# qcNPU/LifeLong-CLIP

Measured on AMD Instinct MI355X. Metric: images/sec/GPU (ViT-B/16 fwd+bwd, bs=256) + online A_AUC on CIFAR-100, higher is better.
Workload: dtype bf16

## Files before the change

include/lc_clip.h:

```cpp
#ifndef LC_CLIP_H
#define LC_CLIP_H
#include <hip/hip_runtime_api.h>
#include <stdint.h>

#ifdef __cplusplus
extern "C" {
#endif

#define LC_OK 0
#define LC_EINVAL (-1)
#define LC_ELAUNCH (-2)
#define LC_EUNSUPPORTED (-3)

#define LC_EPI_BF16 0
#define LC_EPI_F32 1
#define LC_EPI_RESID 2
#define LC_EPI_GELU 3
#define LC_EPI_GELU_BWD 4
#define LC_EPI_BF16_F32 5
#define LC_EPI_GELU_D 6
#define LC_EPI_MUL 7
#define LC_EPI_GELU_D_Q8 12
#define LC_EPI_MUL_Q8 13
#define LC_EPI_RESID16 14
// ... 214 lines not shown
                               const float* beta, void* y, long ldy, float* mean, float* rstd,
                               long row_mul, long row_add);

int lc_adapter_bwd(hipStream_t stream, int M, int D, const void* gout, long ldg, const void* h,
                   const void* WuT, const void* WdT, float scale, float keep, void* dpre,
                   void* dz, long ldz);

int lc_adapter_bwd_set_form(int fused);

int lc_adapter_wgrad(hipStream_t stream, int M, int D, const void* gout, long ldg, const void* h,
                     const void* z, long ldz, const void* dpre, float scale, float* dWu,
                     float* dbu, float* dWd, float* dbd);
int lc_adapter_wgrad_ws(hipStream_t stream, int M, int D, const void* gout, long ldg,
                        const void* h, const void* z, long ldz, const void* dpre, float scale,
                        float* dWu, float* dbu, float* dWd, float* dbd, void* ws, long ws_bytes);

int lc_check_finite(hipStream_t stream, long n, const float* g, int* flag);

int lc_adamw(hipStream_t stream, long n, float* p, const float* g, float* m, float* v, float lr,
             float b1, float b2, float eps, float wd, int step, const int* skip,
             const long long* step_dev);

int lc_counter_add(hipStream_t stream, int n, long long* ctr, long long delta);

int lc_adam_step_advance(hipStream_t stream, long long* ctr, const int* skip);

int lc_l2norm_rows(hipStream_t stream, int R, int E, const float* f, long ldf, float* out,
                   float* norms);

int lc_clip_head(hipStream_t stream, int B, int C, int E, const float* img_n, const float* txt_n,
// ... 66 lines not shown
int lc_adapter_ln_fwd_f16(hipStream_t stream, int M, int D, const void* z, long ldz, const void* Wd,
                          const float* bd, const void* Wu, const float* bu, float scale, float keep,
                          unsigned long long seed, const unsigned long long* seed_dev,
                          const float* resid, float* xout, long ldx, void* hout,
                          const float* gamma, const float* beta, void* y, long ldy, float* mean,
                          float* rstd);
int lc_adapter_bwd_f16(hipStream_t stream, int M, int D, const void* gout, long ldg, const void* h,
                       const void* WuT, const void* WdT, float scale, float keep, void* dpre,
                       void* dz, long ldz);
int lc_adapter_wgrad_f16(hipStream_t stream, int M, int D, const void* gout, long ldg, const void* h,
                         const void* z, long ldz, const void* dpre, float scale, float* dWu,
                         float* dbu, float* dWd, float* dbd);
int lc_adapter_wgrad_ws_f16(hipStream_t stream, int M, int D, const void* gout, long ldg,
                            const void* h, const void* z, long ldz, const void* dpre, float scale,
                            float* dWu, float* dbu, float* dWd, float* dbd, void* ws, long ws_bytes);
int lc_patchify_f16(hipStream_t stream, int n_img, int res, int patch, const float* img, void* out);
int lc_vit_embed_ln_f16(hipStream_t stream, int n_img, int n_patch, int D, const float* patch,
                        const float* cls, const float* pos, const float* ln_pre_w,
                        const float* ln_pre_b, float* x0, const float* ln1_w, const float* ln1_b,
                        void* y, float* mean1, float* rstd1);


int lc_mvp_select(hipStream_t stream, int B, int P, int W, int K, const float* query, long ldq,
                  const float* key, long ldk, const float* count, int64_t* idx, float* dist,
                  float* qnorm, float* knorm, unsigned long long* hist);

int lc_mvp_simloss(hipStream_t stream, int B, int P, int W, int K, int contrastiv,
                   const float* key, long ldk, const float* count, const int64_t* idx,
                   const float* dist, const float* knorm, float* kcos, float* rawgd, float* rawW,
                   float* coef, float* loss);
// ... 44 lines not shown
```

lifelong-clip_amd/csrc/gemm.hip:

```cpp
#include "lc_common.h"
#include <stdlib.h>
#include <type_traits>

enum {
  EPI_BF16 = 0,
  EPI_F32 = 1,
  EPI_RESID = 2,
  EPI_GELU = 3,
  EPI_GELU_BWD = 4,
  EPI_BF16_F32 = 5,
  EPI_GELU_D = 6,
  EPI_MUL = 7,
  EPI_AD_DOWN = 8,
  EPI_AD_UP = 9,
  EPI_AD_MASK = 10,
  EPI_AD_ADD = 11,
  EPI_GELU_D_Q8 = 12,
  EPI_MUL_Q8 = 13,
  EPI_RESID16 = 14,
};

namespace {

constexpr int BK = 64;


LC_DEV int swz(int row, int chunk) { return chunk ^ ((row >> 1) & 7); }

LC_DEV void tile_coords(int tile, int tiles_m, int tiles_n, int gm, int& tm, int& tn) {
  if (gm <= 1) {
    tm = tile / tiles_n;
    tn = tile % tiles_n;
    return;
  }
// ... 249 lines not shown
      } else if constexpr (EPI == EPI_AD_ADD) {
#pragma unroll
        for (int i = 0; i < CPL; ++i) w[i] = bfv(xb, i) + v[i];
        store_bf(rs0, ldo0, m, w);
      }
    }
  }
}

template <int BM, int BN, int WM, int WN, int STAGES, int EPI>
__global__ void __launch_bounds__(64 * WM * WN, (WM * WN == 4 ? 2 : 1))
gemm_nt_kernel(int M, int N, int K, const bf16_t* __restrict__ A, long lda,
               const bf16_t* __restrict__ B, long ldb, const float* __restrict__ bias,
               float alpha, void* __restrict__ out0, long ldo0, void* __restrict__ out1,
               long ldo1, const void* __restrict__ aux, long ldaux, EpiParams ep) {
  constexpr int NW = WM * WN;
  constexpr int TM = BM / WM / 16;
  constexpr int TN = BN / WN / 16;
  constexpr int STAGE_BYTES = (BM + BN) * 128;
  constexpr int LOADS = (BM + BN) / 8 / NW;
  constexpr int PASS_MAX = STAGES == 1 ? 16 : 32;
  constexpr int EPI_BYTES = NW * ((BM / WM) % PASS_MAX == 0 ? PASS_MAX : 16) * (BN / WN + 4) * 4;
  constexpr int SMEM = STAGES * STAGE_BYTES > EPI_BYTES ? STAGES * STAGE_BYTES : EPI_BYTES;
  __shared__ __attribute__((aligned(16))) char smem[SMEM];

  const int tid = threadIdx.x, lane = tid & 63, wave = tid >> 6;
  const int wm = wave / WN, wn = wave % WN;

  const int tiles_n = N / BN;
  const int tiles_m = (M + BM - 1) / BM;
// ... 72 lines not shown

    int cur = 0;
    for (int kt = 0; kt < nk; ++kt) {
      const int pre = kt + STAGES - 1;
      int pbuf = cur + STAGES - 1;
      if (pbuf >= STAGES) pbuf -= STAGES;
      if (pre < nk) stage(pbuf, pre);
      compute(smem + cur * STAGE_BYTES);
      if (pre < nk) wait_vmcnt<LOADS * (STAGES - 2)>();
      else wait_vmcnt<0>();
      __builtin_amdgcn_s_barrier();
      cur = cur + 1 == STAGES ? 0 : cur + 1;
    }
  }

  store_tile<BM, BN, WM, WN, EPI, PASS_MAX>(acc, smem, SMEM, m0, n0, M, bias, alpha, out0, ldo0,
                                            out1, ldo1, aux, ldaux, ep);
}

LC_DEV int swz64(int row, int chunk) { return chunk ^ (((row >> 3) & 1) << 1); }

struct SplitK {
  int dp_tiles;
  int splits;
  float* slabs;
  int* tickets;
};

LC_DEV void splitk_slice(int s_id, int tail_tiles, int S, int& tail, int& split) {
#ifdef LC_SPLITK_SPREAD
  tail = s_id / S;
  split = s_id % S;
// ... 871 lines not shown
        if (n1 < N1 && n2 < N2) atomicAdd(C + (long)n1 * ldc + n2, acc[i][j][r] * alpha);
      }
}

struct TnProb {
  const bf16_t* W;
  long ldw;
  const bf16_t* S;
  long lds;
  float* C;
  long ldc;
  int Nw, ns, trans;
  float alpha;
  float* cs_w;
  float cs_w_scale;
  float* cs_s;
  float cs_s_scale;
  int M, n_chunks, n_tiles, wgs;
  float* part;
  int pw;
  const float* div;
  int w16;
};
LC_DEV float tn_unscale(const TnProb& p, float v) { return p.div ? v / *p.div : v; }

template <int PW>
struct TnGeom {
  static constexpr int ROWB = PW * 2;
  static constexpr int WB = 64 * ROWB;
  static constexpr int SLOT = WB + 64 * 128;
#ifndef TNW256_STAGES
#define TNW256_STAGES 3
#endif
  static constexpr int STAGES = PW == 256 ? TNW256_STAGES : 5;
  static constexpr int WPW = WB / 1024 / 8;
  static constexpr int LOADS = WPW + 1;
  static constexpr int TI = PW / 64;
};

__host__ __device__ inline int tn_pslot(int pw) { return pw * 64 + pw + 64; }

template <int PW>
__global__ void __launch_bounds__(512, 1)
gemm_tn_wide_kernel(TnProb p0, TnProb p1) {
  using Geo = TnGeom<PW>;
  constexpr int STAGES = Geo::STAGES, SLOT = Geo::SLOT, LOADS = Geo::LOADS, TI = Geo::TI;
  constexpr int ROWB = Geo::ROWB, LPRW = ROWB / 16, RPP = 64 / LPRW;
  constexpr int PSLOT = PW * 64 + PW + 64;
  __shared__ __attribute__((aligned(16))) char smem[STAGES * SLOT];
  const bool second = (int)blockIdx.x >= p0.wgs;
  const TnProb& p = second ? p1 : p0;
  const int bid = second ? blockIdx.x - p0.wgs : blockIdx.x;
  const int tid = threadIdx.x, lane = tid & 63;
  const int wave = __builtin_amdgcn_readfirstlane(tid >> 6);
  const int wn = wave & 3, wsv = wave >> 2;
  const int g = lane >> 4, t = lane & 15;
  const int tile = bid % p.n_tiles, cidx = bid / p.n_tiles;
  const int nblk = (p.M + 63) / 64;
  float* slot = p.part ? p.part + (long)(tile * p.n_chunks + cidx) * PSLOT : nullptr;
  if (cidx >= nblk) {
    if (slot)
      for (int e = tid; e < PSLOT; e += 512) slot[e] = 0.f;
    return;
  }
  const int nsteps = (nblk - 1 - cidx) / p.n_chunks + 1;
  auto blk_row = [&](int s) { return (cidx + s * p.n_chunks) * 64; };
  const int nw_pad = (p.Nw + 63) & ~63;
  const bool do_csw = p.cs_w != nullptr && wsv == 0;
  const bool do_css = p.cs_s != nullptr && tile == 0 && wn == 0;

  auto dma = [&](int s) {
    char* sl = smem + (s % STAGES) * SLOT;
    const int r0 = blk_row(s);
#pragma unroll
    for (int i = 0; i < Geo::WPW; ++i) {
      const int piece = wave * Geo::WPW + i;
      const int lr = piece * RPP + lane / LPRW;
      const int pc = lane % LPRW;
      const int c = (((pc >> 1) ^ swz_w(lr)) << 1) | (pc & 1);
      const int r = min(r0 + lr, p.M - 1);
      int col = tile * PW + c * 8;
      col = col < nw_pad ? col : col - 64;
      glds16(p.W + (long)r * p.ldw + col, sl + piece * 1024);
    }
    {
      const int piece = wave;
      const int lr = piece * 8 + (lane >> 3);
      const int pc = lane & 7;
      const int c = (((pc >> 1) ^ swz_s(lr)) << 1) | (pc & 1);
      const int r = min(r0 + lr, p.M - 1);
      glds16(p.S + (long)r * p.lds + c * 8, sl + Geo::WB + piece * 1024);
    }
  };

  f32x4 acc[TI][2], csw[TI], css[2];
#pragma unroll
  for (int i = 0; i < TI; ++i) {
    csw[i] = f32x4{0.f, 0.f, 0.f, 0.f};
#pragma unroll
    for (int j = 0; j < 2; ++j) acc[i][j] = f32x4{0.f, 0.f, 0.f, 0.f};
  }
  css[0] = css[1] = f32x4{0.f, 0.f, 0.f, 0.f};
  const short one = LC_ONE16;

#pragma unroll
  for (int s = 0; s < STAGES - 1; ++s)
    if (s < nsteps) dma(s);
  for (int s = 0; s < nsteps; ++s) {
    const int ahead = min(nsteps - 1 - s, STAGES - 2);
    if (STAGES > 4 && ahead >= 3) wait_vmcnt<3 * LOADS>();
    else if (STAGES > 3 && ahead == 2) wait_vmcnt<2 * LOADS>();
    else if (ahead >= 1) wait_vmcnt<LOADS>();
    else wait_vmcnt<0>();
    lds_barrier();
    if (s + STAGES - 1 < nsteps) dma(s + STAGES - 1);
    const uint32_t sw = lds_addr(smem + (s % STAGES) * SLOT);
    const uint32_t ss = sw + Geo::WB;
    const int valid = p.M - blk_row(s);
    bf16x8 fwk[2][TI], fsk[2][2];
#pragma unroll
    for (int ks = 0; ks < 2; ++ks) {
      const int row = ks * 32 + g * 8 + (t >> 2);
#pragma unroll
      for (int i = 0; i < TI; ++i)
        fwk[ks][i] = tr_frag_asm<ROWB>(sw, row, wn * (PW / 4) + i * 16 + (t & 3) * 4);
#pragma unroll
      for (int j = 0; j < 2; ++j)
        fsk[ks][j] = tr_frag_asm<128>(ss, row, wsv * 32 + j * 16 + (t & 3) * 4);
    }
    lds_wait0();
    if (p.w16) {
// ... 148 lines not shown
    LC_NT_CASE(EPI_RESID)
    LC_NT_CASE(EPI_RESID16)
    LC_NT_CASE(EPI_GELU)
    LC_NT_CASE(EPI_GELU_BWD)
    LC_NT_CASE(EPI_BF16_F32)
    LC_NT_CASE(EPI_GELU_D)
    LC_NT_CASE(EPI_MUL)
    LC_NT_CASE(EPI_AD_DOWN)
    LC_NT_CASE(EPI_AD_UP)
    LC_NT_CASE(EPI_AD_MASK)
    LC_NT_CASE(EPI_AD_ADD)
    default:
      return LC_EINVAL;
  }
#undef LC_NT_CASE
  LC_LAUNCH_RET();
}

int g_split_mode = -1;

int cu_count() {
  static int cus[64] = {0};
  int dev = 0;
  if (hipGetDevice(&dev) != hipSuccess || dev < 0 || dev >= 64) return 256;
  if (cus[dev] == 0) {
    int n = 0;
    if (hipDeviceGetAttribute(&n, hipDeviceAttributeMultiprocessorCount, dev) != hipSuccess || n <= 0)
      n = 256;
    cus[dev] = n;
  }
// ... 392 lines not shown
  LC_CHECK_ARG(bias == nullptr || ((uintptr_t)bias & 15) == 0);
  if ((epi != EPI_BF16 && epi != EPI_F32) || alpha != 1.0f) return LC_EUNSUPPORTED;
  const FullRoute r = full_route(epi, bias, alpha, M_full, N, K, ws, ws_bytes);
  if (!r.ok) return LC_EUNSUPPORTED;
  const int S = r.sk.splits, nt = K / 64;
  const int tiles = ((M_full + 255) / 256) * (N / 256);
  float* part = nullptr;
  if (S > 1) {
    if (LC_SPLITK_TICKET_BYTES + (long)S * n * N * 4 > ws_bytes) return LC_EUNSUPPORTED;
    part = reinterpret_cast<float*>(static_cast<char*>(ws) + LC_SPLITK_TICKET_BYTES);
  }
  const EpiParams ep{nullptr, 0, 1.0f, 1.0f, 0, g_dbg};
  int rc = lc_gemm_nt_ex(stream, epi, n, N, K, A, lda, B, ldb, bias, alpha, out, ldo, nullptr, 0,
                         nullptr, 0, ep, nullptr, 0);
  if (rc != LC_OK || S == 1) return rc;
  for (int s = 0; s < S; ++s) {
    const int tb = s * nt / S, te = (s + 1) * nt / S;
    rc = lc_gemm_nt_ex(stream, EPI_F32, n, N, (te - tb) * 64,
                       static_cast<const bf16_t*>(A) + (long)tb * 64, lda,
                       static_cast<const bf16_t*>(B) + (long)tb * 64, ldb, nullptr, 1.0f,
                       part + (long)s * n * N, N, nullptr, 0, nullptr, 0, ep, nullptr, 0);
    if (rc != LC_OK) return rc;
  }
  dim3 grid(tiles - r.sk.dp_tiles), block(256);
  if (epi == EPI_BF16)
    hipLaunchKernelGGL((gemm_rows_fixup_kernel<EPI_BF16>), grid, block, 0, stream, n, N, M_full,
                       mul, add, r.group_m, r.sk.dp_tiles, S, part, bias, alpha, out, ldo);
  else
    hipLaunchKernelGGL((gemm_rows_fixup_kernel<EPI_F32>), grid, block, 0, stream, n, N, M_full,
                       mul, add, r.group_m, r.sk.dp_tiles, S, part, bias, alpha, out, ldo);
  LC_LAUNCH_RET();
}

int lc_gemm_nt(hipStream_t stream, int epi, int M, int N, int K, const void* A, long lda,
               const void* B, long ldb, const float* bias, float alpha, void* out0, long ldo0,
               void* out1, long ldo1, const void* aux, long ldaux) {
  return lc_gemm_nt_ws(stream, epi, M, N, K, A, lda, B, ldb, bias, alpha, out0, ldo0, out1, ldo1,
                       aux, ldaux, nullptr, 0);
// ... 116 lines not shown
                     static_cast<const bf16_t*>(A), lda, static_cast<const bf16_t*>(B), ldb, alpha,
                     C, ldc, colsum, colsum_scale);
  LC_LAUNCH_RET();
}

int lc_adapter_wgrad(hipStream_t stream, int M, int D, const void* gout, long ldg, const void* h,
                     const void* z, long ldz, const void* dpre, float scale, float* dWu,
                     float* dbu, float* dWd, float* dbd) {
  return lc_adapter_wgrad_ws(stream, M, D, gout, ldg, h, z, ldz, dpre, scale, dWu, dbu, dWd, dbd,
                             nullptr, 0);
}

static int adapter_wgrad(hipStream_t stream, int M, int D, const void* gout, long ldg,
                         const void* h, const void* z, long ldz, const void* dpre, float scale,
                         float* dWu, float* dbu, float* dWd, float* dbd, void* ws, long ws_bytes,
                         const float* div, int g16 = 0) {
  LC_CHECK_ARG(M > 0 && D > 0 && D % 64 == 0 && ldg % 8 == 0 && ldz % 8 == 0 && ldg >= D &&
               ldz >= D);
  LC_CHECK_ARG(dWu != nullptr && dWd != nullptr);
  TnProb up{}, down{};
  up.div = down.div = div;
  up.W = static_cast<const bf16_t*>(gout);
  up.w16 = g16;
  up.ldw = ldg;
  up.S = static_cast<const bf16_t*>(h);
  up.lds = 64;
  up.C = dWu;
  up.ldc = 64;
  up.Nw = D;
  up.ns = 64;
  up.trans = 0;
// ... 17 lines not shown
  down.cs_s = dbd;
  down.cs_s_scale = 1.0f;
  down.pw = pw;
  down.M = M;
  down.n_tiles = (D + pw - 1) / pw;
  plan_tn(up, 2 * up.n_tiles);
  plan_tn(down, 2 * down.n_tiles);
#ifdef LC_DIAG_SKIP_WGRAD
  return LC_OK;
#endif
  const long need = (long)(up.wgs + down.wgs) * tn_pslot(pw) * 4;
  if (ws != nullptr && ws_bytes >= LC_SPLITK_TICKET_BYTES + need) {
    up.part = reinterpret_cast<float*>(static_cast<char*>(ws) + LC_SPLITK_TICKET_BYTES);
    down.part = up.part + (long)up.wgs * tn_pslot(pw);
  }
  if (pw == 256)
    hipLaunchKernelGGL(gemm_tn_wide_kernel<256>, dim3(up.wgs + down.wgs), dim3(512), 0, stream, up,
                       down);
  else
    hipLaunchKernelGGL(gemm_tn_wide_kernel<128>, dim3(up.wgs + down.wgs), dim3(512), 0, stream, up,
                       down);
  if (up.part) {
    const int outs = 2 * (D * 64 + D + 64);
    hipLaunchKernelGGL(tn_reduce_kernel, dim3((outs + 255) / 256), dim3(256), 0, stream, up, down);
  }
  LC_LAUNCH_RET();
}

int lc_adapter_wgrad_ws(hipStream_t stream, int M, int D, const void* gout, long ldg,
                        const void* h, const void* z, long ldz, const void* dpre, float scale,
                        float* dWu, float* dbu, float* dWd, float* dbd, void* ws, long ws_bytes) {
  return adapter_wgrad(stream, M, D, gout, ldg, h, z, ldz, dpre, scale, dWu, dbu, dWd, dbd, ws,
                       ws_bytes, nullptr);
}

#ifndef LC_F16
int lc_adapter_wgrad_ws_unscaled(hipStream_t stream, int M, int D, const void* gout, long ldg,
                                 const void* h, const void* z, long ldz, const void* dpre,
                                 float scale, float* dWu, float* dbu, float* dWd, float* dbd,
                                 void* ws, long ws_bytes, const float* gscale) {
  LC_CHECK_ARG(gscale != nullptr);
  return adapter_wgrad(stream, M, D, gout, ldg, h, z, ldz, dpre, scale, dWu, dbu, dWd, dbd, ws,
                       ws_bytes, gscale);
}

int lc_adapter_wgrad_ws_unscaled_g16(hipStream_t stream, int M, int D, const void* gout, long ldg,
                                     const void* h, const void* z, long ldz, const void* dpre,
                                     float scale, float* dWu, float* dbu, float* dWd, float* dbd,
                                     void* ws, long ws_bytes, const float* gscale) {
  LC_CHECK_ARG(gscale != nullptr);
  return adapter_wgrad(stream, M, D, gout, ldg, h, z, ldz, dpre, scale, dWu, dbu, dWd, dbd, ws,
// ... 6 lines not shown
```

lifelong-clip_amd/csrc/lc_f16_names.h:

```cpp
#pragma once
#define lc_attn_fwd lc_attn_fwd_f16
#define lc_attn_bwd_fp8 lc_attn_bwd_fp8_f16
#define lc_attn_bwd lc_attn_bwd_f16
#define lc_attn_bwd_set_form lc_attn_bwd_set_form_f16
#define lc_attn_row_fwd lc_attn_row_fwd_f16
#define lc_attn_row_bwd lc_attn_row_bwd_f16
#define lc_attn_bwd_live_row lc_attn_bwd_live_row_f16
#define lc_gemm_nt_ex lc_gemm_nt_ex_f16
#define lc_gemm_nt lc_gemm_nt_f16
#define lc_gemm_nt_ws lc_gemm_nt_ws_f16
#define lc_gemm_nt_rows lc_gemm_nt_rows_f16
#define lc_gemm_split_plan lc_gemm_split_plan_f16
#define lc_gemm_set_debug lc_gemm_set_debug_f16
#define lc_gemm_nt_fp8 lc_gemm_nt_fp8_f16
#define lc_gemm_set_tile lc_gemm_set_tile_f16
#define lc_gemm_set_streamk lc_gemm_set_streamk_f16
#define lc_gemm_tn lc_gemm_tn_f16
#define lc_gemm_tn_ws lc_gemm_tn_ws_f16
#define lc_adapter_wgrad lc_adapter_wgrad_f16
#define lc_adapter_wgrad_ws lc_adapter_wgrad_ws_f16
#define lc_layernorm_fwd lc_layernorm_fwd_f16
#define lc_layernorm_fwd_fp8 lc_layernorm_fwd_fp8_f16
#define lc_layernorm_bwd lc_layernorm_bwd_f16
#define lc_layernorm_bwd_fp8 lc_layernorm_bwd_fp8_f16
#define lc_patchify lc_patchify_f16
#define lc_vit_assemble lc_vit_assemble_f16
#define lc_vit_embed_ln lc_vit_embed_ln_f16
#define lc_text_embed lc_text_embed_f16
#define lc_eot_rows lc_eot_rows_f16
#define lc_cast_bf16 lc_cast_bf16_f16
#define lc_merge_weight lc_merge_weight_f16
#define lc_cast_weights_bf16 lc_cast_weights_bf16_f16
#define lc_merge_weights_bf16 lc_merge_weights_bf16_f16
#define lc_lora_grad lc_lora_grad_f16
#define lc_lora_grad_ws lc_lora_grad_ws_f16
// ... 11 lines not shown
```

lifelong-clip_amd/lcclip/_lib.py:

```python
from __future__ import annotations

import ctypes
import os
from ctypes import c_float, c_int, c_long, c_ulonglong, c_void_p

import torch

_HERE = os.path.dirname(os.path.abspath(__file__))
LIB_PATH = os.path.join(_HERE, "liblcclip.so")

P = c_void_p
SIGNATURES = {
    "lc_gemm_nt": [P, c_int, c_int, c_int, c_int, P, c_long, P, c_long, P, c_float, P, c_long, P,
                   c_long, P, c_long],
    "lc_gemm_nt_ws": [P, c_int, c_int, c_int, c_int, P, c_long, P, c_long, P, c_float, P, c_long,
                      P, c_long, P, c_long, P, c_long],
    "lc_gemm_nt_rows": [P, c_int, c_int, c_int, c_int, P, c_long, P, c_long, P, c_float, P, c_long,
                        c_int, c_long, c_long, P, c_long],
    "lc_gemm_split_plan": [c_int, c_int, c_int, c_long, P, P],
    "lc_gemm_nt_fp8": [P, c_int, c_int, c_int, c_int, P, c_long, P, c_long, P, c_long, P, c_long,
                       P, c_float, P, c_long, P, c_long, P, c_long, P, c_long, P, c_long],
    "lc_quant_fp8": [P, c_long, c_int, P, c_int, c_long, c_long, P, c_long, P, c_long],
    "lc_gemm_set_tile": [c_int],
    "lc_gemm_set_streamk": [c_int],
# ... 34 lines not shown
    "lc_lora_grad_ws": [P, c_int, c_int, c_int, c_int, P, c_long, P, c_long, P, c_long, P, c_long,
                        c_float, P, P, P, c_long],
    "lc_adapter_fwd": [P, c_int, c_int, P, c_long, P, P, P, P, c_float, c_float, c_ulonglong, P, P,
                       P, c_long, P],
    "lc_adapter_ln_fwd": [P, c_int, c_int, P, c_long, P, P, P, P, c_float, c_float, c_ulonglong,
                          P, P, P, c_long, P, P, P, P, c_long, P, P],
    "lc_adapter_fwd_rows": [P, c_int, c_int, P, c_long, P, P, P, P, c_float, c_float, c_ulonglong,
                            P, P, P, c_long, P, c_long, c_long],
    "lc_adapter_ln_fwd_rows": [P, c_int, c_int, P, c_long, P, P, P, P, c_float, c_float,
                               c_ulonglong, P, P, P, c_long, P, P, P, P, c_long, P, P, c_long,
                               c_long],
    "lc_adapter_bwd": [P, c_int, c_int, P, c_long, P, P, P, c_float, c_float, P, P, c_long],
    "lc_adapter_wgrad": [P, c_int, c_int, P, c_long, P, P, c_long, P, c_float, P, P, P, P],
    "lc_adapter_wgrad_ws": [P, c_int, c_int, P, c_long, P, P, c_long, P, c_float, P, P, P, P, P,
                            c_long],
    "lc_check_finite": [P, c_long, P, P],
    "lc_adamw": [P, c_long, P, P, P, P, c_float, c_float, c_float, c_float, c_float, c_int, P, P],
    "lc_counter_add": [P, c_int, P, c_long],
    "lc_adam_step_advance": [P, P, P],
    "lc_l2norm_rows": [P, c_int, c_int, P, c_long, P, P],
    "lc_clip_head": [P, c_int, c_int, c_int, P, P, P, P, P, P, P],
    "lc_head_logits": [P, c_int, c_int, c_int, P, P, P, P, P],
    "lc_softmax_bwd_rows": [P, c_int, c_int, P, P, P],
    "lc_head_feat_grad": [P, c_int, c_int, c_int, P, c_long, c_long, P, P, P, P, P, P],
    "lc_grad_pow2_normalize": [P, c_long, P, P, c_int],
    "lc_add_unscaled": [P, c_long, P, P, P],
    "lc_mvp_select": [P, c_int, c_int, c_int, c_int, P, c_long, P, c_long, P, P, P, P, P, P],
    "lc_mvp_simloss": [P, c_int, c_int, c_int, c_int, c_int, P, c_long, P, P, P, P, P, P, P, P, P],
    "lc_mvp_simloss_bwd": [P, c_int, c_int, c_int, c_int, c_int, P, c_long, P, c_long, P, P, P, P,
                           P, P, P, P, P, P, c_long],
# ... 8 lines not shown
    "lc_mvp_afs": [P, c_int, c_int, P, P, P, P, P],
    "lc_mvp_head_bwd": [P, c_int, c_int, c_int, P, P, P, P, c_long, P, P, c_float, P, P, c_long],
    "lc_device_cu_count": [c_int, P],
    "lc_stream_create_cumask": [c_int, c_int, c_int, c_int, P],
    "lc_stream_destroy": [P],
}

F16_ENTRY_POINTS = ("lc_gemm_nt", "lc_gemm_nt_ws", "lc_gemm_nt_rows", "lc_gemm_tn", "lc_gemm_tn_ws",
                    "lc_layernorm_fwd", "lc_layernorm_bwd", "lc_attn_fwd", "lc_attn_bwd",
                    "lc_attn_bwd_set_form", "lc_attn_row_fwd", "lc_attn_row_bwd",
                    "lc_attn_bwd_live_row",
                    "lc_adapter_fwd_rows", "lc_adapter_ln_fwd_rows",
                    "lc_cast_bf16", "lc_merge_weight", "lc_cast_weights_bf16",
                    "lc_merge_weights_bf16", "lc_lora_grad", "lc_lora_grad_ws", "lc_adapter_fwd",
                    "lc_adapter_ln_fwd", "lc_adapter_bwd", "lc_adapter_wgrad",
                    "lc_adapter_wgrad_ws", "lc_patchify", "lc_vit_embed_ln")
SIGNATURES.update({n + "_f16": SIGNATURES[n] for n in F16_ENTRY_POINTS})
SIGNATURES.update({n + "_x16": SIGNATURES[n] for n in (
    "lc_layernorm_fwd", "lc_layernorm_bwd", "lc_vit_embed_ln", "lc_adapter_ln_fwd",
    "lc_adapter_ln_fwd_rows", "lc_layernorm_fwd_fp8", "lc_layernorm_bwd_fp8")})
SIGNATURES["lc_layernorm_bwd_g16"] = SIGNATURES["lc_layernorm_bwd"]
SIGNATURES["lc_adapter_wgrad_ws_unscaled"] = SIGNATURES["lc_adapter_wgrad_ws"] + [P]
SIGNATURES["lc_adapter_wgrad_ws_unscaled_g16"] = SIGNATURES["lc_adapter_wgrad_ws_unscaled"]
SIGNATURES["lc_adapter_bwd_g16"] = SIGNATURES["lc_adapter_bwd"]
SIGNATURES["lc_lora_grad_ws_unscaled"] = SIGNATURES["lc_lora_grad_ws"] + [P]

_lib = None


class LcError(RuntimeError):
    pass


def load(path: str = None):
    global _lib
    if _lib is not None:
        return _lib
    if path is None:
# ... 39 lines not shown
```

lifelong-clip_amd/lcclip/engine.py:

```python
from __future__ import annotations

import itertools
import os
from collections import namedtuple
from contextlib import nullcontext
from types import SimpleNamespace

import torch

from . import ops
from .ops import BF16, F16, F32, EPI_BF16, EPI_F32, EPI_GELU, EPI_GELU_D, EPI_MUL, EPI_RESID
from .ops import EPI_RESID16
from .ops import EPI_GELU_D_Q8, EPI_MUL_Q8

_seed_counter = itertools.count(1)


def _empty(shape, dtype, dev):
    return None if dtype is None else torch.empty(shape, dtype=dtype, device=dev)


def _rows(t, n):
    return None if t is None else t[:n]

# ... 651 lines not shown
                                             ox, oxb, bufs.q_mat(Mx), dres=dx_mid[:Mx]))
        else:
            bufs.set_q(None)
            ops.layernorm_bwd(dh[:Mx], s.x_in, s.mean1, s.rstd1, blk.ln_1.weight, ox, oxb,
                              dres=dres1)
        return True

    def _adapter_bwd(self, c, blk, st, gout, h, z, keep, dz, pad=None):
        ad = blk.adaptmlp
        M = gout.shape[0]
        dpre = _empty((M, ad.down_size), self.dt, gout.device)
        ops.adapter_bwd(gout, h, st.wuT, st.wdT, ad.scale, keep, dpre, dz)
        with c.side():
            if c.gs is not None:
                dpre.record_stream(c.gs)
            if pad is not None:
                gout, h, z, dpre = self._wgrad_rows(*pad, gout, h, z, dpre)
            ops.adapter_wgrad(gout, h, z, dpre, ad.scale, *(c.grad(p) for p in (
                ad.up_proj.weight, ad.up_proj.bias, ad.down_proj.weight, ad.down_proj.bias)),
                gscale=c.gscale)
        return dz

    ROWS_EXACT = os.environ.get("LCCLIP_ROWS_EXACT", "1") != "0"
    ROW_BWD = os.environ.get("LCCLIP_ROW_BWD", "0") == "1"

    def rows_ok(self):
        return self.variant == "adapter" and self.precision == "bf16"

    @staticmethod
    def _spread(src, n, L, dst=None, fill=0):
        if dst is None:
            dst = torch.empty((n * L, src.shape[1]), dtype=src.dtype, device=src.device)
        elif _same_storage(src, dst):
            src = src.clone()
        if fill is not None:
# ... 15 lines not shown
            full = out.new_empty((Mx, out.shape[1])) if scratch is None else scratch[:Mx]
            self._gemm(st, name, self._spread(A, n_seq, L, dst=buf[:Mx]), epi, full, **kw)
            self._gather(full, n_seq, L, out)

    def _attn_bwd_rows(self, s, dO, dqkv, n_seq, L, da, dh):
        H, Mx = self.n_head, n_seq * L
        args = (s.qkv, s.O, dO, s.lse, dqkv, n_seq, L, H, 0, self.causal)
        if self.ROW_BWD:
            ops.attn_row_bwd(*args)
        elif not (self.ROWS_EXACT and ops.attn_bwd_live_row(*args)):
            Of = self._spread(s.O, n_seq, L, dst=dh[:Mx])
            dOf = self._spread(dO, n_seq, L, dst=da.view(-1)[:Mx * dO.shape[1]].view(Mx, -1))
            lsef = self._spread(s.lse.view(-1, 1), n_seq * H, L, fill=1e30).view(-1, L)
            ops.attn_bwd(s.qkv, Of, dOf, lsef, dqkv, n_seq, L, H, self.causal)

    def _wgrad_rows(self, n_seq, L, *operands):
        return operands if self.ROW_BWD else tuple(self._spread(t, n_seq, L) for t in operands)

    HALF_GRAD_DIRECT = os.environ.get("LCCLIP_HALF_GRAD_DIRECT", "1") != "0"

    def half_grad_direct(self):
        return self.variant == "adapter" and self.HALF_GRAD_DIRECT

    PROMPT_KEEP = os.environ.get("LCCLIP_PROMPT_KEEP", "1") != "0"
    MERGE_BATCH = os.environ.get("LCCLIP_MERGE_BATCH", "1") != "0"
    LORA_1P = os.environ.get("LCCLIP_LORA_1P", "1") != "0"

    def _lora_1p(self, r, K, N):
        return self.LORA_1P and r <= 4 and (K, N) in ((768, 2304), (768, 768), (512, 1536),
                                                      (512, 512))

    def lora_half_grad_ok(self):
# ... 398 lines not shown
```

lifelong-clip_amd/lcclip/ops.py:

```python
from __future__ import annotations

import ctypes

import torch

from ._lib import LcError, call, load, ptr, stream_of

BF16 = torch.bfloat16
F16 = torch.float16
F32 = torch.float32
HALF = (BF16, F16)

EPI_BF16, EPI_F32, EPI_RESID, EPI_GELU, EPI_GELU_BWD, EPI_BF16_F32, EPI_GELU_D, EPI_MUL = range(8)
EPI_RESID16 = 14
EPI_GELU_D_Q8, EPI_MUL_Q8 = 12, 13


def _rowmajor(t, dtype, name):
    if (t.dtype not in HALF) if dtype == HALF else (t.dtype != dtype):
        raise TypeError(f"{name}: expected {dtype}, got {t.dtype}")
    if t.dim() != 2 or t.stride(1) != 1:
        raise ValueError(f"{name}: expected a 2-D row-major view, got shape {tuple(t.shape)} "
                         f"strides {t.stride()}")

# ... 515 lines not shown
        if any(t is not None and t.dtype == F16 for t in ts):
            raise TypeError(f"{name}: a float16 gout takes bf16 partners")
        if gout.stride(-1) != 1 or gout.stride(0) % 8 or gout.data_ptr() % 16:
            raise ValueError(f"{name}: half gout must be row-major, 16-B aligned, row stride % 8")
        return name + "_g16"
    return _sym16(name, gout, *ts)


def adapter_bwd(gout, h, WuT, WdT, scale, keep, dpre, dz):
    M, D = gout.shape
    call(_g16("lc_adapter_bwd", gout, h, WuT, WdT, dpre, dz), stream_of(gout), M, D, ptr(gout),
         gout.stride(0), ptr(h), ptr(WuT), ptr(WdT), float(scale), float(keep), ptr(dpre),
         ptr(dz), dz.stride(0) if dz is not None else D)


def adapter_wgrad(gout, h, z, dpre, scale, dWu, dbu, dWd, dbd, gscale=None):
    M, D = gout.shape
    for t, name in ((gout, "gout"), (z, "z")):
        _rowmajor(t, HALF, name)
    for t, name in ((h, "h"), (dpre, "dpre")):
        if t.dtype not in HALF or not t.is_contiguous() or t.shape != (M, 64):
            raise ValueError(f"{name} must be contiguous 16-bit [M, 64]")
    if z.shape != (M, D) or dWu.shape != (D, 64) or dWd.shape != (64, D):
        raise ValueError("adapter_wgrad shape mismatch")
    for t in (dWu, dWd, dbu, dbd):
        if t is not None and (t.dtype != F32 or not t.is_contiguous()):
            raise ValueError("gradient buffers must be contiguous f32")
    ws = splitk_workspace(torch.cuda.current_stream(gout.device))
    if gscale is not None:
        name = _g16("lc_adapter_wgrad_ws_unscaled", gout, h, z, dpre)
        if (h.dtype != BF16 or z.dtype != BF16 or dpre.dtype != BF16 or gscale.dtype != F32
                or gscale.numel() != 1):
            raise TypeError("adapter_wgrad: gscale takes bf16 partners and an f32 device scalar")
        call(name, stream_of(gout), M, D, ptr(gout), gout.stride(0),
             ptr(h), ptr(z), z.stride(0), ptr(dpre), float(scale), ptr(dWu), ptr(dbu), ptr(dWd),
             ptr(dbd), ptr(ws), ws.numel(), ptr(gscale))
        return
    if gout.dtype != h.dtype:
        raise TypeError("adapter_wgrad: a float16 gout beside bf16 operands needs its gscale")
    call(_sym16("lc_adapter_wgrad_ws", gout, h, z, dpre), stream_of(gout), M, D, ptr(gout), gout.stride(0), ptr(h), ptr(z),
         z.stride(0), ptr(dpre), float(scale), ptr(dWu), ptr(dbu), ptr(dWd), ptr(dbd), ptr(ws),
         ws.numel())


def check_finite(g, flag):
    call("lc_check_finite", stream_of(g), g.numel(), ptr(g), ptr(flag))


def adamw(p, g, m, v, lr, b1, b2, eps, wd, step, skip=None, step_dev=None):
    call("lc_adamw", stream_of(p), p.numel(), ptr(p), ptr(g), ptr(m), ptr(v), float(lr), float(b1),
         float(b2), float(eps), float(wd), int(step), ptr(skip), ptr(step_dev))


def counter_add(ctr, delta=1):
    if ctr.dtype != torch.int64 or not ctr.is_contiguous():
        raise ValueError("counters must be a contiguous int64 tensor")
    call("lc_counter_add", stream_of(ctr), ctr.numel(), ptr(ctr), int(delta))
# ... 288 lines not shown
```

Baseline: 10590.

## Compute adapter wgrad directly over strided live rows instead of spreading operands

Adds a rows-aware variant of the adapter weight-gradient TN kernel. It reads only the live rows (index = i*mul+add), zero-fills the dead rows, and skips fully dead 64-row blocks in its pipelined loads. This removes the separate spread/scatter of gout, h, z and dpre into full-size buffers before wgrad. It also folds the per-slice split-K NT GEMM loop into one launch with a grid.y slice dimension, to cut launch overhead. The costs are more complex DMA scheduling with extra per-row index math, and a fallback path to the old spread when the new entry point is missing.

```diff
diff --git a/include/lc_clip.h b/include/lc_clip.h
--- a/include/lc_clip.h
+++ b/include/lc_clip.h
@@ -252,6 +252,20 @@
 int lc_adapter_wgrad_ws(hipStream_t stream, int M, int D, const void* gout, long ldg,
                         const void* h, const void* z, long ldz, const void* dpre, float scale,
                         float* dWu, float* dbu, float* dWd, float* dbd, void* ws, long ws_bytes);
+int lc_adapter_wgrad_rows_ws(hipStream_t stream, int n, int D, const void* gout, long ldg,
+                             const void* h, const void* z, long ldz, const void* dpre,
+                             float scale, float* dWu, float* dbu, float* dWd, float* dbd,
+                             int M_full, long mul, long add, void* ws, long ws_bytes);
+int lc_adapter_wgrad_rows_ws_unscaled(hipStream_t stream, int n, int D, const void* gout, long ldg,
+                                      const void* h, const void* z, long ldz, const void* dpre,
+                                      float scale, float* dWu, float* dbu, float* dWd, float* dbd,
+                                      int M_full, long mul, long add, void* ws, long ws_bytes,
+                                      const float* gscale);
+int lc_adapter_wgrad_rows_ws_unscaled_g16(hipStream_t stream, int n, int D, const void* gout,
+                                          long ldg, const void* h, const void* z, long ldz,
+                                          const void* dpre, float scale, float* dWu, float* dbu,
+                                          float* dWd, float* dbd, int M_full, long mul, long add,
+                                          void* ws, long ws_bytes, const float* gscale);
 
 int lc_check_finite(hipStream_t stream, long n, const float* g, int* flag);
 
@@ -348,6 +362,10 @@
 int lc_adapter_wgrad_ws_f16(hipStream_t stream, int M, int D, const void* gout, long ldg,
                             const void* h, const void* z, long ldz, const void* dpre, float scale,
                             float* dWu, float* dbu, float* dWd, float* dbd, void* ws, long ws_bytes);
+int lc_adapter_wgrad_rows_ws_f16(hipStream_t stream, int n, int D, const void* gout, long ldg,
+                                 const void* h, const void* z, long ldz, const void* dpre,
+                                 float scale, float* dWu, float* dbu, float* dWd, float* dbd,
+                                 int M_full, long mul, long add, void* ws, long ws_bytes);
 int lc_patchify_f16(hipStream_t stream, int n_img, int res, int patch, const float* img, void* out);
 int lc_vit_embed_ln_f16(hipStream_t stream, int n_img, int n_patch, int D, const float* patch,
                         const float* cls, const float* pos, const float* ln_pre_w,
diff --git a/lifelong-clip_amd/csrc/gemm.hip b/lifelong-clip_amd/csrc/gemm.hip
--- a/lifelong-clip_amd/csrc/gemm.hip
+++ b/lifelong-clip_amd/csrc/gemm.hip
@@ -18,6 +18,7 @@
   EPI_GELU_D_Q8 = 12,
   EPI_MUL_Q8 = 13,
   EPI_RESID16 = 14,
+  EPI_F32_SLICES = 15,
 };
 
 namespace {
@@ -297,6 +298,14 @@
                const bf16_t* __restrict__ B, long ldb, const float* __restrict__ bias,
                float alpha, void* __restrict__ out0, long ldo0, void* __restrict__ out1,
                long ldo1, const void* __restrict__ aux, long ldaux, EpiParams ep) {
+  if constexpr (EPI == EPI_F32_SLICES) {
+    const int nt = K / BK, s = blockIdx.y, S = gridDim.y;
+    const int tb = s * nt / S, te = (s + 1) * nt / S;
+    A += tb * BK;
+    B += tb * BK;
+    K = (te - tb) * BK;
+    out0 = static_cast<float*>(out0) + (long)s * M * ldo0;
+  }
   constexpr int NW = WM * WN;
   constexpr int TM = BM / WM / 16;
   constexpr int TN = BN / WN / 16;
@@ -399,8 +408,8 @@
     }
   }
 
-  store_tile<BM, BN, WM, WN, EPI, PASS_MAX>(acc, smem, SMEM, m0, n0, M, bias, alpha, out0, ldo0,
-                                            out1, ldo1, aux, ldaux, ep);
+  store_tile<BM, BN, WM, WN, EPI == EPI_F32_SLICES ? EPI_F32 : EPI, PASS_MAX>(
+      acc, smem, SMEM, m0, n0, M, bias, alpha, out0, ldo0, out1, ldo1, aux, ldaux, ep);
 }
 
 LC_DEV int swz64(int row, int chunk) { return chunk ^ (((row >> 3) & 1) << 1); }
@@ -1302,14 +1311,18 @@
   float alpha;
   float* cs_w;
   float cs_w_scale;
+  int rows_n;
   float* cs_s;
   float cs_s_scale;
   int M, n_chunks, n_tiles, wgs;
+  int rows_mul;
   float* part;
   int pw;
+  int rows_add;
   const float* div;
   int w16;
 };
+static_assert(sizeof(TnProb) == 144, "the rows_* fields sit in TnProb's padding");
 LC_DEV float tn_unscale(const TnProb& p, float v) { return p.div ? v / *p.div : v; }
 
 template <int PW>
@@ -1328,9 +1341,14 @@
 
 __host__ __device__ inline int tn_pslot(int pw) { return pw * 64 + pw + 64; }
 
-template <int PW>
+constexpr int TN_ROWS = 1;
+static __device__ uint4 tn_zero16 = {0, 0, 0, 0};
+
+template <int PWF>
 __global__ void __launch_bounds__(512, 1)
 gemm_tn_wide_kernel(TnProb p0, TnProb p1) {
+  constexpr int PW = PWF & ~TN_ROWS;
+  constexpr bool ROWS = (PWF & TN_ROWS) != 0;
   using Geo = TnGeom<PW>;
   constexpr int STAGES = Geo::STAGES, SLOT = Geo::SLOT, LOADS = Geo::LOADS, TI = Geo::TI;
   constexpr int ROWB = Geo::ROWB, LPRW = ROWB / 16, RPP = 64 / LPRW;
@@ -1357,8 +1375,17 @@
   const bool do_csw = p.cs_w != nullptr && wsv == 0;
   const bool do_css = p.cs_s != nullptr && tile == 0 && wn == 0;
 
-  auto dma = [&](int s) {
-    char* sl = smem + (s % STAGES) * SLOT;
+  auto live_row = [&](int r) {
+    const int d = r - p.rows_add;
+    return d >= 0 && d % p.rows_mul == 0 && d / p.rows_mul < p.rows_n ? d / p.rows_mul : -1;
+  };
+  auto live_blk = [&](int s) {
+    const int lo = blk_row(s);
+    const int i0 = lo <= p.rows_add ? 0 : (lo - p.rows_add + p.rows_mul - 1) / p.rows_mul;
+    return i0 < p.rows_n && i0 * p.rows_mul + p.rows_add < lo + 64;
+  };
+  auto dma = [&](int s, int q) {
+    char* sl = smem + (q % STAGES) * SLOT;
     const int r0 = blk_row(s);
 #pragma unroll
     for (int i = 0; i < Geo::WPW; ++i) {
@@ -1369,7 +1396,14 @@
       const int r = min(r0 + lr, p.M - 1);
       int col = tile * PW + c * 8;
       col = col < nw_pad ? col : col - 64;
-      glds16(p.W + (long)r * p.ldw + col, sl + piece * 1024);
+      if constexpr (ROWS) {
+        const int ci = live_row(r);
+        const void* src = &tn_zero16;
+        if (ci >= 0) src = p.W + (long)ci * p.ldw + col;
+        glds16(src, sl + piece * 1024);
+      } else {
+        glds16(p.W + (long)r * p.ldw + col, sl + piece * 1024);
+      }
     }
     {
       const int piece = wave;
@@ -1377,7 +1411,14 @@
       const int pc = lane & 7;
       const int c = (((pc >> 1) ^ swz_s(lr)) << 1) | (pc & 1);
       const int r = min(r0 + lr, p.M - 1);
-      glds16(p.S + (long)r * p.lds + c * 8, sl + Geo::WB + piece * 1024);
+      if constexpr (ROWS) {
+        const int ci = live_row(r);
+        const void* src = &tn_zero16;
+        if (ci >= 0) src = p.S + (long)ci * p.lds + c * 8;
+        glds16(src, sl + Geo::WB + piece * 1024);
+      } else {
+        glds16(p.S + (long)r * p.lds + c * 8, sl + Geo::WB + piece * 1024);
+      }
     }
   };
 
@@ -1391,18 +1432,29 @@
   css[0] = css[1] = f32x4{0.f, 0.f, 0.f, 0.f};
   const short one = LC_ONE16;
 
-#pragma unroll
-  for (int s = 0; s < STAGES - 1; ++s)
-    if (s < nsteps) dma(s);
+  int issued = 0, next = 0, q = 0;
+  auto dma_next_live = [&]() {
+    while (next < nsteps && !live_blk(next)) ++next;
+    if (next < nsteps) dma(next++, issued++);
+  };
+#pragma unroll
+  for (int s = 0; s < STAGES - 1; ++s) {
+    if constexpr (ROWS) dma_next_live();
+    else if (s < nsteps) dma(s, s);
+  }
   for (int s = 0; s < nsteps; ++s) {
-    const int ahead = min(nsteps - 1 - s, STAGES - 2);
+    if constexpr (ROWS) {
+      if (!live_blk(s)) continue;
+    }
+    const int ahead = ROWS ? issued - 1 - q : min(nsteps - 1 - s, STAGES - 2);
     if (STAGES > 4 && ahead >= 3) wait_vmcnt<3 * LOADS>();
     else if (STAGES > 3 && ahead == 2) wait_vmcnt<2 * LOADS>();
     else if (ahead >= 1) wait_vmcnt<LOADS>();
     else wait_vmcnt<0>();
     lds_barrier();
-    if (s + STAGES - 1 < nsteps) dma(s + STAGES - 1);
-    const uint32_t sw = lds_addr(smem + (s % STAGES) * SLOT);
+    if constexpr (ROWS) dma_next_live();
+    else if (s + STAGES - 1 < nsteps) dma(s + STAGES - 1, s + STAGES - 1);
+    const uint32_t sw = lds_addr(smem + ((ROWS ? q++ : s) % STAGES) * SLOT);
     const uint32_t ss = sw + Geo::WB;
     const int valid = p.M - blk_row(s);
     bf16x8 fwk[2][TI], fsk[2][2];
@@ -1581,6 +1633,18 @@
       return LC_EINVAL;
   }
 #undef LC_NT_CASE
+  LC_LAUNCH_RET();
+}
+
+template <int BM, int BN, int WM, int WN, int STAGES>
+int launch_nt_slices(hipStream_t st, int M, int N, int nt, int S, const bf16_t* A, long lda,
+                     const bf16_t* B, long ldb, float* out, const EpiParams& ep) {
+  LC_CHECK_ARG(lda < (1L << 22) && ldb < (1L << 22));
+  dim3 grid(((M + BM - 1) / BM) * (N / BN), S), block(64 * WM * WN);
+  hipLaunchKernelGGL((gemm_nt_kernel<BM, BN, WM, WN, STAGES, EPI_F32_SLICES>), grid, block, 0, st,
+                     M, N, nt * 64, A, lda, B, ldb, static_cast<const float*>(nullptr), 1.0f,
+                     static_cast<void*>(out), (long)N, static_cast<void*>(nullptr), 0L,
+                     static_cast<const void*>(nullptr), 0L, ep);
   LC_LAUNCH_RET();
 }
 
@@ -2003,14 +2067,25 @@
   int rc = lc_gemm_nt_ex(stream, epi, n, N, K, A, lda, B, ldb, bias, alpha, out, ldo, nullptr, 0,
                          nullptr, 0, ep, nullptr, 0);
   if (rc != LC_OK || S == 1) return rc;
-  for (int s = 0; s < S; ++s) {
-    const int tb = s * nt / S, te = (s + 1) * nt / S;
-    rc = lc_gemm_nt_ex(stream, EPI_F32, n, N, (te - tb) * 64,
-                       static_cast<const bf16_t*>(A) + (long)tb * 64, lda,
-                       static_cast<const bf16_t*>(B) + (long)tb * 64, ldb, nullptr, 1.0f,
-                       part + (long)s * n * N, N, nullptr, 0, nullptr, 0, ep, nullptr, 0);
-    if (rc != LC_OK) return rc;
-  }
+  int fam = route_tile(0, EPI_F32, n, N, (nt / S) * 64);
+  for (int s = 0; s < S; ++s)
+    if (route_tile(0, EPI_F32, n, N, ((s + 1) * nt / S - s * nt / S) * 64) != fam) fam = -1;
+  const bf16_t* a = static_cast<const bf16_t*>(A);
+  const bf16_t* b = static_cast<const bf16_t*>(B);
+  if (fam == 1)
+    rc = launch_nt_slices<128, 128, 2, 2, 2>(stream, n, N, nt, S, a, lda, b, ldb, part, ep);
+  else if (fam == 4)
+    rc = launch_nt_slices<128, 64, 4, 1, 2>(stream, n, N, nt, S, a, lda, b, ldb, part, ep);
+  else if (fam == 11)
+    rc = launch_nt_slices<128, 64, 4, 1, 1>(stream, n, N, nt, S, a, lda, b, ldb, part, ep);
+  else
+    for (int s = 0; s < S && rc == LC_OK; ++s) {
+      const int tb = s * nt / S, te = (s + 1) * nt / S;
+      rc = lc_gemm_nt_ex(stream, EPI_F32, n, N, (te - tb) * 64, a + (long)tb * 64, lda,
+                         b + (long)tb * 64, ldb, nullptr, 1.0f, part + (long)s * n * N, N,
+                         nullptr, 0, nullptr, 0, ep, nullptr, 0);
+    }
+  if (rc != LC_OK) return rc;
   dim3 grid(tiles - r.sk.dp_tiles), block(256);
   if (epi == EPI_BF16)
     hipLaunchKernelGGL((gemm_rows_fixup_kernel<EPI_BF16>), grid, block, 0, stream, n, N, M_full,
@@ -2157,7 +2232,7 @@
 static int adapter_wgrad(hipStream_t stream, int M, int D, const void* gout, long ldg,
                          const void* h, const void* z, long ldz, const void* dpre, float scale,
                          float* dWu, float* dbu, float* dWd, float* dbd, void* ws, long ws_bytes,
-                         const float* div, int g16 = 0) {
+                         const float* div, int g16 = 0, const int* rows = nullptr) {
   LC_CHECK_ARG(M > 0 && D > 0 && D % 64 == 0 && ldg % 8 == 0 && ldz % 8 == 0 && ldg >= D &&
                ldz >= D);
   LC_CHECK_ARG(dWu != nullptr && dWd != nullptr);
@@ -2205,7 +2280,18 @@
     up.part = reinterpret_cast<float*>(static_cast<char*>(ws) + LC_SPLITK_TICKET_BYTES);
     down.part = up.part + (long)up.wgs * tn_pslot(pw);
   }
-  if (pw == 256)
+  if (rows != nullptr) {
+    if (!up.part) return LC_EUNSUPPORTED;
+    up.rows_n = down.rows_n = rows[0];
+    up.rows_mul = down.rows_mul = rows[1];
+    up.rows_add = down.rows_add = rows[2];
+    if (pw == 256)
+      hipLaunchKernelGGL(gemm_tn_wide_kernel<256 | TN_ROWS>, dim3(up.wgs + down.wgs), dim3(512), 0,
+                         stream, up, down);
+    else
+      hipLaunchKernelGGL(gemm_tn_wide_kernel<128 | TN_ROWS>, dim3(up.wgs + down.wgs), dim3(512), 0,
+                         stream, up, down);
+  } else if (pw == 256)
     hipLaunchKernelGGL(gemm_tn_wide_kernel<256>, dim3(up.wgs + down.wgs), dim3(512), 0, stream, up,
                        down);
   else
@@ -2225,7 +2311,48 @@
                        ws_bytes, nullptr);
 }
 
+static int adapter_wgrad_rows(hipStream_t stream, int n, int D, const void* gout, long ldg,
+                              const void* h, const void* z, long ldz, const void* dpre,
+                              float scale, float* dWu, float* dbu, float* dWd, float* dbd,
+                              int M_full, long mul, long add, void* ws, long ws_bytes,
+                              const float* div, int g16) {
+  LC_CHECK_ARG(n > 0 && M_full > 0 && M_full <= (1 << 30) && mul >= 1 && mul <= (1L << 30) &&
+               add >= 0 && (long)(n - 1) * mul + add < (long)M_full);
+  LC_CHECK_ARG(ws == nullptr || ((uintptr_t)ws & 255) == 0);
+  const int rows[3] = {n, (int)mul, (int)add};
+  return adapter_wgrad(stream, M_full, D, gout, ldg, h, z, ldz, dpre, scale, dWu, dbu, dWd, dbd,
+                       ws, ws_bytes, div, g16, rows);
+}
+
+int lc_adapter_wgrad_rows_ws(hipStream_t stream, int n, int D, const void* gout, long ldg,
+                             const void* h, const void* z, long ldz, const void* dpre,
+                             float scale, float* dWu, float* dbu, float* dWd, float* dbd,
+                             int M_full, long mul, long add, void* ws, long ws_bytes) {
+  return adapter_wgrad_rows(stream, n, D, gout, ldg, h, z, ldz, dpre, scale, dWu, dbu, dWd, dbd,
+                            M_full, mul, add, ws, ws_bytes, nullptr, 0);
+}
+
 #ifndef LC_F16
+int lc_adapter_wgrad_rows_ws_unscaled(hipStream_t stream, int n, int D, const void* gout, long ldg,
+                                      const void* h, const void* z, long ldz, const void* dpre,
+                                      float scale, float* dWu, float* dbu, float* dWd, float* dbd,
+                                      int M_full, long mul, long add, void* ws, long ws_bytes,
+                                      const float* gscale) {
+  LC_CHECK_ARG(gscale != nullptr);
+  return adapter_wgrad_rows(stream, n, D, gout, ldg, h, z, ldz, dpre, scale, dWu, dbu, dWd, dbd,
+                            M_full, mul, add, ws, ws_bytes, gscale, 0);
+}
+
+int lc_adapter_wgrad_rows_ws_unscaled_g16(hipStream_t stream, int n, int D, const void* gout,
+                                          long ldg, const void* h, const void* z, long ldz,
+                                          const void* dpre, float scale, float* dWu, float* dbu,
+                                          float* dWd, float* dbd, int M_full, long mul, long add,
+                                          void* ws, long ws_bytes, const float* gscale) {
+  LC_CHECK_ARG(gscale != nullptr);
+  return adapter_wgrad_rows(stream, n, D, gout, ldg, h, z, ldz, dpre, scale, dWu, dbu, dWd, dbd,
+                            M_full, mul, add, ws, ws_bytes, gscale, 1);
+}
+
 int lc_adapter_wgrad_ws_unscaled(hipStream_t stream, int M, int D, const void* gout, long ldg,
                                  const void* h, const void* z, long ldz, const void* dpre,
                                  float scale, float* dWu, float* dbu, float* dWd, float* dbd,
diff --git a/lifelong-clip_amd/csrc/lc_f16_names.h b/lifelong-clip_amd/csrc/lc_f16_names.h
--- a/lifelong-clip_amd/csrc/lc_f16_names.h
+++ b/lifelong-clip_amd/csrc/lc_f16_names.h
@@ -19,6 +19,7 @@
 #define lc_gemm_tn_ws lc_gemm_tn_ws_f16
 #define lc_adapter_wgrad lc_adapter_wgrad_f16
 #define lc_adapter_wgrad_ws lc_adapter_wgrad_ws_f16
+#define lc_adapter_wgrad_rows_ws lc_adapter_wgrad_rows_ws_f16
 #define lc_layernorm_fwd lc_layernorm_fwd_f16
 #define lc_layernorm_fwd_fp8 lc_layernorm_fwd_fp8_f16
 #define lc_layernorm_bwd lc_layernorm_bwd_f16
diff --git a/lifelong-clip_amd/lcclip/_lib.py b/lifelong-clip_amd/lcclip/_lib.py
--- a/lifelong-clip_amd/lcclip/_lib.py
+++ b/lifelong-clip_amd/lcclip/_lib.py
@@ -72,6 +72,8 @@
     "lc_adapter_wgrad": [P, c_int, c_int, P, c_long, P, P, c_long, P, c_float, P, P, P, P],
     "lc_adapter_wgrad_ws": [P, c_int, c_int, P, c_long, P, P, c_long, P, c_float, P, P, P, P, P,
                             c_long],
+    "lc_adapter_wgrad_rows_ws": [P, c_int, c_int, P, c_long, P, P, c_long, P, c_float, P, P, P, P,
+                                 c_int, c_long, c_long, P, c_long],
     "lc_check_finite": [P, c_long, P, P],
     "lc_adamw": [P, c_long, P, P, P, P, c_float, c_float, c_float, c_float, c_float, c_int, P, P],
     "lc_counter_add": [P, c_int, P, c_long],
@@ -110,7 +112,8 @@
                     "lc_cast_bf16", "lc_merge_weight", "lc_cast_weights_bf16",
                     "lc_merge_weights_bf16", "lc_lora_grad", "lc_lora_grad_ws", "lc_adapter_fwd",
                     "lc_adapter_ln_fwd", "lc_adapter_bwd", "lc_adapter_wgrad",
-                    "lc_adapter_wgrad_ws", "lc_patchify", "lc_vit_embed_ln")
+                    "lc_adapter_wgrad_ws", "lc_adapter_wgrad_rows_ws", "lc_patchify",
+                    "lc_vit_embed_ln")
 SIGNATURES.update({n + "_f16": SIGNATURES[n] for n in F16_ENTRY_POINTS})
 SIGNATURES.update({n + "_x16": SIGNATURES[n] for n in (
     "lc_layernorm_fwd", "lc_layernorm_bwd", "lc_vit_embed_ln", "lc_adapter_ln_fwd",
@@ -118,6 +121,8 @@
 SIGNATURES["lc_layernorm_bwd_g16"] = SIGNATURES["lc_layernorm_bwd"]
 SIGNATURES["lc_adapter_wgrad_ws_unscaled"] = SIGNATURES["lc_adapter_wgrad_ws"] + [P]
 SIGNATURES["lc_adapter_wgrad_ws_unscaled_g16"] = SIGNATURES["lc_adapter_wgrad_ws_unscaled"]
+SIGNATURES["lc_adapter_wgrad_rows_ws_unscaled"] = SIGNATURES["lc_adapter_wgrad_rows_ws"] + [P]
+SIGNATURES["lc_adapter_wgrad_rows_ws_unscaled_g16"] = SIGNATURES["lc_adapter_wgrad_rows_ws_unscaled"]
 SIGNATURES["lc_adapter_bwd_g16"] = SIGNATURES["lc_adapter_bwd"]
 SIGNATURES["lc_lora_grad_ws_unscaled"] = SIGNATURES["lc_lora_grad_ws"] + [P]
 
diff --git a/lifelong-clip_amd/lcclip/engine.py b/lifelong-clip_amd/lcclip/engine.py
--- a/lifelong-clip_amd/lcclip/engine.py
+++ b/lifelong-clip_amd/lcclip/engine.py
@@ -689,11 +689,12 @@
         with c.side():
             if c.gs is not None:
                 dpre.record_stream(c.gs)
+            grads = [c.grad(p) for p in (ad.up_proj.weight, ad.up_proj.bias, ad.down_proj.weight,
+                                         ad.down_proj.bias)]
             if pad is not None:
-                gout, h, z, dpre = self._wgrad_rows(*pad, gout, h, z, dpre)
-            ops.adapter_wgrad(gout, h, z, dpre, ad.scale, *(c.grad(p) for p in (
-                ad.up_proj.weight, ad.up_proj.bias, ad.down_proj.weight, ad.down_proj.bias)),
-                gscale=c.gscale)
+                self._wgrad_rows(*pad, (gout, h, z, dpre), ad.scale, grads, c.gscale)
+            else:
+                ops.adapter_wgrad(gout, h, z, dpre, ad.scale, *grads, gscale=c.gscale)
         return dz
 
     ROWS_EXACT = os.environ.get("LCCLIP_ROWS_EXACT", "1") != "0"
@@ -739,8 +740,13 @@
             lsef = self._spread(s.lse.view(-1, 1), n_seq * H, L, fill=1e30).view(-1, L)
             ops.attn_bwd(s.qkv, Of, dOf, lsef, dqkv, n_seq, L, H, self.causal)
 
-    def _wgrad_rows(self, n_seq, L, *operands):
-        return operands if self.ROW_BWD else tuple(self._spread(t, n_seq, L) for t in operands)
+    def _wgrad_rows(self, n_seq, L, operands, scale, grads, gscale):
+        if self.ROW_BWD:
+            ops.adapter_wgrad(*operands, scale, *grads, gscale=gscale)
+        elif not (self.ROWS_EXACT and ops.adapter_wgrad_rows(
+                *operands, scale, *grads, n_seq * L, L, 0, gscale=gscale)):
+            ops.adapter_wgrad(*(self._spread(t, n_seq, L) for t in operands), scale, *grads,
+                              gscale=gscale)
 
     HALF_GRAD_DIRECT = os.environ.get("LCCLIP_HALF_GRAD_DIRECT", "1") != "0"
 
diff --git a/lifelong-clip_amd/lcclip/ops.py b/lifelong-clip_amd/lcclip/ops.py
--- a/lifelong-clip_amd/lcclip/ops.py
+++ b/lifelong-clip_amd/lcclip/ops.py
@@ -553,7 +553,7 @@
          ptr(dz), dz.stride(0) if dz is not None else D)
 
 
-def adapter_wgrad(gout, h, z, dpre, scale, dWu, dbu, dWd, dbd, gscale=None):
+def _adapter_wgrad(gout, h, z, dpre, scale, dWu, dbu, dWd, dbd, gscale, rows, ws):
     M, D = gout.shape
     for t, name in ((gout, "gout"), (z, "z")):
         _rowmajor(t, HALF, name)
@@ -565,21 +565,39 @@
     for t in (dWu, dWd, dbu, dbd):
         if t is not None and (t.dtype != F32 or not t.is_contiguous()):
             raise ValueError("gradient buffers must be contiguous f32")
-    ws = splitk_workspace(torch.cuda.current_stream(gout.device))
+    base = "lc_adapter_wgrad_ws" if rows is None else "lc_adapter_wgrad_rows_ws"
     if gscale is not None:
-        name = _g16("lc_adapter_wgrad_ws_unscaled", gout, h, z, dpre)
+        name = _g16(base + "_unscaled", gout, h, z, dpre)
         if (h.dtype != BF16 or z.dtype != BF16 or dpre.dtype != BF16 or gscale.dtype != F32
                 or gscale.numel() != 1):
             raise TypeError("adapter_wgrad: gscale takes bf16 partners and an f32 device scalar")
-        call(name, stream_of(gout), M, D, ptr(gout), gout.stride(0),
-             ptr(h), ptr(z), z.stride(0), ptr(dpre), float(scale), ptr(dWu), ptr(dbu), ptr(dWd),
-             ptr(dbd), ptr(ws), ws.numel(), ptr(gscale))
-        return
-    if gout.dtype != h.dtype:
-        raise TypeError("adapter_wgrad: a float16 gout beside bf16 operands needs its gscale")
-    call(_sym16("lc_adapter_wgrad_ws", gout, h, z, dpre), stream_of(gout), M, D, ptr(gout), gout.stride(0), ptr(h), ptr(z),
-         z.stride(0), ptr(dpre), float(scale), ptr(dWu), ptr(dbu), ptr(dWd), ptr(dbd), ptr(ws),
-         ws.numel())
+    else:
+        if gout.dtype != h.dtype:
+            raise TypeError("adapter_wgrad: a float16 gout beside bf16 operands needs its gscale")
+        name = _sym16(base, gout, h, z, dpre)
+    fn = getattr(load(), name) if rows is None else getattr(load(), name, None)
+    if rows is not None and (fn is None or fn.argtypes is None):
+        return EUNSUPPORTED
+    args = (stream_of(gout), M, D, ptr(gout), gout.stride(0), ptr(h), ptr(z), z.stride(0),
+            ptr(dpre), float(scale), ptr(dWu), ptr(dbu), ptr(dWd), ptr(dbd),
+            *(() if rows is None else rows), ptr(ws), ws.numel() if ws is not None else 0,
+            *(() if gscale is None else (ptr(gscale),)))
+    rc = fn(*args)
+    if rc != 0 and not (rows is not None and rc == EUNSUPPORTED):
+        raise LcError(f"{name} returned {rc}")
+    return rc
+
+
+def adapter_wgrad(gout, h, z, dpre, scale, dWu, dbu, dWd, dbd, gscale=None):
+    ws = splitk_workspace(torch.cuda.current_stream(gout.device))
+    _adapter_wgrad(gout, h, z, dpre, scale, dWu, dbu, dWd, dbd, gscale, None, ws)
+
+
+def adapter_wgrad_rows(gout, h, z, dpre, scale, dWu, dbu, dWd, dbd, M_full, mul, add=0,
+                       gscale=None, workspace=True):
+    ws = splitk_workspace(torch.cuda.current_stream(gout.device)) if workspace else None
+    return _adapter_wgrad(gout, h, z, dpre, scale, dWu, dbu, dWd, dbd, gscale,
+                          (int(M_full), int(mul), int(add)), ws) == 0
 
 
 def check_finite(g, flag):
diff --git a/profiles/wgrad_rows/compare.py b/profiles/wgrad_rows/compare.py
--- /dev/null
+++ b/profiles/wgrad_rows/compare.py
@@ -0,0 +1,36 @@
+import json
+import sys
+
+import numpy as np
+
+out = sys.argv[1]
+
+
+def leg(name):
+    line = [l for l in open(f"{out}/bench.{name}.log") if l.startswith("{")][-1]
+    r = json.loads(line)
+    return r["ms_per_step"], r["value"], np.load(f"{out}/dump.{name}/loss.npy"), \
+        np.load(f"{out}/dump.{name}/probs.npy")
+
+
+tree = [leg(f"tree.{i}") for i in (1, 2, 3)]
+parent = [leg(f"parent.{i}") for i in (1, 2, 3)]
+exact0 = leg("exact0")
+for name, runs in (("tree", tree), ("parent library", parent), ("LCCLIP_ROWS_EXACT=0", [exact0])):
+    ms = [r[0] for r in runs]
+    print(f"{name}: ms per step {', '.join(f'{m:.3f}' for m in ms)}; images/s "
+          f"{', '.join(f'{r[1]:.1f}' for r in runs)}; mean {np.mean(ms):.3f} ms; "
+          f"max - min {max(ms) - min(ms):.3f} ms")
+mt, mp = np.mean([r[0] for r in tree]), np.mean([r[0] for r in parent])
+spread = max(max(r[0] for r in runs) - min(r[0] for r in runs) for runs in (tree, parent))
+print(f"tree - parent: {mt - mp:+.3f} ms per step ({(mp / mt - 1) * 100:+.2f} % images/s); "
+      f"{(mp - mt) / spread:.1f} x the larger spread ({spread:.3f} ms); a gain needs more than 3")
+p0 = parent[0][3].view(np.uint32)
+probs_ok = all(np.array_equal(r[3].view(np.uint32), p0) for r in tree + parent + [exact0])
+print("probs bit-identical to the parent's in every run:", probs_ok)
+pl = [float(r[2]) for r in parent]
+tl = [float(r[2]) for r in tree]
+print("loss, parent runs:", pl, "tree runs:", tl, "ROWS_EXACT=0:", float(exact0[2]))
+loss_ok = all(min(pl) <= t <= max(pl) for t in tl)
+print(f"parent's own loss spread {max(pl) - min(pl):.3g}; tree's losses inside it: {loss_ok}")
+sys.exit(0 if probs_ok and loss_ok else 1)
```

After: 10660, median of 6. About the same (+0.6%).
